# mrvollger/rustybam

Hardware: NVIDIA B200
Metric: lifted window-records/s (higher is better)
Workload: dtype u32/u64 (+f32 identities)

## Files before the change

### rustybam_b200/csrc/rb_kernels.cu

```cuda
#include <algorithm>
#include <cstdio>

#include "f32_fmt.cuh"
#include "lift_core.cuh"
#include "rb_kernels.cuh"
#include "rec_core.cuh"
#include "stream_core.cuh"

namespace rb {

__device__ __forceinline__ uint4 ld_nc_v4(const void* p) {
    uint4 r;
    asm volatile("ld.global.nc.L1::no_allocate.v4.u32 {%0,%1,%2,%3}, [%4];" : "=r"(r.x), "=r"(r.y), "=r"(r.z), "=r"(r.w) : "l"(p));
    return r;
}
__device__ __forceinline__ unsigned long long ld_volatile_u64(const unsigned long long* p) {
    unsigned long long v;
    asm volatile("ld.volatile.global.u64 %0, [%1];" : "=l"(v) : "l"(p));
    return v;
}
__device__ __forceinline__ uint32_t ld_volatile_u32(const uint32_t* p) {
    uint32_t v;
    asm volatile("ld.volatile.global.u32 %0, [%1];" : "=r"(v) : "l"(p));
    return v;
// ... 428 lines not shown
            __threadfence();
            x = payload_load(st == 2u ? &pre[idx] : &agg[idx]);
        }
        const unsigned stopm = __ballot_sync(0xffffffffu, st == 2u || x.flag);
        const int stop = stopm ? (__ffs(stopm) - 1) : 31;
        if (lane > stop) x = seg_identity();
#pragma unroll
        for (int d = 1; d < 32; d <<= 1) {
            const SegVal y = seg_shfl(x, (lane + d) & 31);
            if (lane + d < 32) x = seg_combine(y, x);
        }
        const SegVal tot = seg_shfl(x, 0);
        acc = seg_combine(tot, acc);
        if (stopm) break;
        look -= 32;
        if (look < 0) break;
    }
    if (lane == 0) {
        const SegVal incl = seg_combine(acc, mine);
        payload_store(&pre[b], incl);
        __threadfence();
        atomicExch(&state[b], 2u);
    }
    return acc;
}

__device__ __forceinline__ void st_b128(void* p, uint32_t a, uint32_t b, uint32_t c, uint32_t d) {
    const unsigned long long lo = ((unsigned long long)b << 32) | a, hi = ((unsigned long long)d << 32) | c;
    asm volatile("{\n .reg .b128 r;\n mov.b128 r, {%1, %2};\n st.relaxed.gpu.global.b128 [%0], r;\n}" ::"l"(p), "l"(lo), "l"(hi) : "memory");
}
__device__ __forceinline__ uint4 ld_b128(const void* p) {
    unsigned long long lo, hi;
    asm volatile("{\n .reg .b128 r;\n ld.relaxed.gpu.global.b128 r, [%2];\n mov.b128 {%0, %1}, r;\n}" : "=l"(lo), "=l"(hi) : "l"(p) : "memory");
    return make_uint4((uint32_t)lo, (uint32_t)(lo >> 32), (uint32_t)hi, (uint32_t)(hi >> 32));
}
__device__ __forceinline__ void slot_store(ScanPayload* slot, const SegVal& v, uint32_t tag) {
    const uint32_t* in = reinterpret_cast<const uint32_t*>(&v);
    const uint32_t aux = (in[11] & ~SUB_ABS) | (v.flag ? SUB_ABS : 0u);
    uint4* o = reinterpret_cast<uint4*>(slot);
    st_b128(o + 0, in[0], in[1], in[2], tag);
    st_b128(o + 1, in[3], in[4], in[5], tag);
    st_b128(o + 2, in[6], in[7], in[8], tag);
    st_b128(o + 3, in[9], in[10], aux, tag);
}
__device__ __forceinline__ uint32_t slot_load(const ScanPayload* slot, SegVal& v) {
    const uint4* p = reinterpret_cast<const uint4*>(slot);
    const uint4 a = ld_b128(p + 0), b = ld_b128(p + 1), c = ld_b128(p + 2), d = ld_b128(p + 3);
    if (a.w != b.w || b.w != c.w || c.w != d.w) return 0u;
    uint32_t* out = reinterpret_cast<uint32_t*>(&v);
    out[0] = a.x; out[1] = a.y; out[2] = a.z; out[3] = b.x; out[4] = b.y; out[5] = b.z;
    out[6] = c.x; out[7] = c.y; out[8] = c.z; out[9] = d.x; out[10] = d.y;
    out[11] = d.z & ~SUB_ABS;
    v.flag = (d.z & SUB_ABS) ? 1u : 0u;
    return a.w;
}
__device__ __forceinline__ SegVal lookback_seg2(ScanPayload* slots, uint64_t b, const SegVal& mine) {
    const int lane = threadIdx.x & 31;
    SegVal acc = seg_identity();
    if (b == 0) {
        if (lane == 0) slot_store(&slots[0], mine, 2u);
        return acc;
    }
    if (lane == 0) slot_store(&slots[b], mine, 1u);
    long long look = (long long)b - 1;
    for (;;) {
        const long long idx = look - lane;
        uint32_t st = 2u;
        SegVal x = seg_identity();
        if (idx >= 0) {
            do { st = slot_load(&slots[idx], x); } while (st == 0u);
        }
        const unsigned stopm = __ballot_sync(0xffffffffu, st == 2u || x.flag);
        const int stop = stopm ? (__ffs(stopm) - 1) : 31;
        if (lane > stop) x = seg_identity();
#pragma unroll
        for (int d = 1; d < 32; d <<= 1) {
            const SegVal y = seg_shfl(x, (lane + d) & 31);
            if (lane + d < 32) x = seg_combine(y, x);
        }
        const SegVal tot = seg_shfl(x, 0);
        acc = seg_combine(tot, acc);
        if (stopm) break;
        look -= 32;
        if (look < 0) break;
    }
    if (lane == 0) slot_store(&slots[b], seg_combine(acc, mine), 2u);
    return acc;
}

struct WinStaged {
    const uint32_t* s_ps;
    const uint32_t* s_pe;
    uint32_t js0, je0;
    __device__ __forceinline__ uint32_t ps(uint32_t j) const { return s_ps[j - js0]; }
    __device__ __forceinline__ uint32_t pe(uint32_t j) const { return s_pe[j - je0]; }
};
__device__ __forceinline__ void store_half(void* dst, const void* src) {
    const uint4* s4 = reinterpret_cast<const uint4*>(src);
    uint4* d4 = reinterpret_cast<uint4*>(dst);
#pragma unroll
    for (int k = 0; k < 4; k++) d4[k] = s4[k];
}

template <bool LIFT>
__global__ void __launch_bounds__(SMP_THREADS, LIFT ? 2 : RB_SMP_MINB)
k_scan_lift(const uint32_t* __restrict__ ops, const uint64_t* __restrict__ n_ops_dev, const uint32_t* __restrict__ heads,
            Ctr* __restrict__ samples, uint32_t* blk_state, ScanPayload* blk_agg, ScanPayload* blk_pre, unsigned int* ticket,
            LiftArgs la) {
    extern __shared__ __align__(16) uint32_t s_dyn[];
// ... 199 lines not shown
            SegRec sr;
            sr.eo0 = R.eo0; sr.eo1 = R.eo1; sr.wlo = R.wlo; sr.whi = R.whi;
            sr.s_lo = sr.e_lo = sr.wlo; sr.s_hi = sr.e_hi = sr.whi;
            if (sr.whi > sr.wlo) {
                sr.pair0 = la.pair_off[la.rec_rank[r]];
                const WinGlobal wg{la.w_st, la.w_en, R.t_st, R.t_en};
                uint32_t Tseg = 0;
                for (int j = jb; j < je; j++) {
                    const uint32_t w = my_ops[j];
                    if (is_ref(op_code(w))) Tseg += op_len(w);
                }
                stream_segment(v, sr, wg, k0, (uint32_t)(je - jb), [&](uint32_t j) { return my_ops[jb + (int)j]; }, base, Tseg, acc,
                               [&](uint64_t p, const HalfS& hh) { store_half(&la.hs[p], &hh); },
                               [&](uint64_t p, const HalfE& hh) { store_half(&la.he[p], &hh); });
            }
        }
        if (je >= nvalid) break;
        jb = je;
        r++;
        base = ctr_zero();
    }
}

#ifndef RB_SMP2_MINB
#define RB_SMP2_MINB 4
#endif
#ifndef RB_SMP2_MINB_NOSUBS
#define RB_SMP2_MINB_NOSUBS 5
#endif
template <bool LOCAL, bool NOSUBS = false>
__global__ void __launch_bounds__(SMP_THREADS, NOSUBS ? RB_SMP2_MINB_NOSUBS : RB_SMP2_MINB)
k_samples2(const uint32_t* __restrict__ ops, const uint64_t* __restrict__ n_ops_dev, const uint32_t* __restrict__ heads,
           Ctr* __restrict__ samples, uint32_t* blk_state, ScanPayload* blk_agg, ScanPayload* blk_pre, unsigned int* ticket,
           uint32_t no_subs_arg ) {
    const bool no_subs = NOSUBS || no_subs_arg != 0u;
    static_assert(SAMPLE == 32u, "k_samples2 walks 32-op chunks");
    extern __shared__ __align__(16) uint32_t s_dyn2[];
    uint4* s_ops4 = reinterpret_cast<uint4*>(s_dyn2);
    uint32_t* s_acc = s_dyn2 + SMP_THREADS * SAMPLE;
    __shared__ SegVal s_warp[SMP_THREADS / 32];
    __shared__ SegVal s_blk;
    __shared__ unsigned int s_b;
    const int tid = threadIdx.x, lane = tid & 31, warp = tid >> 5;
    const uint64_t n_ops = *n_ops_dev;
    if (!LOCAL) {
        if (tid == 0) s_b = atomicAdd(ticket, 1u);
        __syncthreads();
    }
    const uint64_t b = LOCAL ? (uint64_t)blockIdx.x : (uint64_t)s_b;
    const uint64_t op0 = b * (uint64_t)SMP_OPS;
    if (op0 >= n_ops && !(n_ops == 0 && b == 0)) {
        if (LOCAL && tid == 0) payload_store(&blk_agg[b], seg_identity());
        return;
    }

    {
        const uint4* src = reinterpret_cast<const uint4*>(ops + op0);
#pragma unroll
        for (int i = 0; i < (int)SAMPLE / 4; i++) {
            const uint32_t v4 = (uint32_t)i * SMP_THREADS + tid;
            uint4 x = make_uint4(0u, 0u, 0u, 0u);
            if (op0 + (uint64_t)v4 * 4u < n_ops) x = src[v4];
            const uint32_t row = v4 >> 3, u = v4 & 7u;
            s_ops4[row * 8u + (u ^ (row & 7u))] = x;
        }
    }
    __syncthreads();

    const uint64_t chunk = b * SMP_THREADS + tid;
    const uint64_t first = chunk << SAMPLE_LOG2;
    int nvalid = 0;
    if (first < n_ops) nvalid = (n_ops - first) < SAMPLE ? (int)(n_ops - first) : (int)SAMPLE;
    const uint32_t h = nvalid ? heads[first >> 5] : 0u;
    const uint32_t sw = (uint32_t)tid & 7u;
    const uint4* row = s_ops4 + (uint32_t)tid * 8u;
    auto op_at = [&](int j) { return reinterpret_cast<const uint32_t*>(&row[((uint32_t)j >> 2) ^ sw])[j & 3]; };
    uint32_t prev_code = 99u;
    if (nvalid) {
        if (tid > 0) prev_code = op_code(s_ops4[(uint32_t)(tid - 1) * 8u + (7u ^ ((uint32_t)(tid - 1) & 7u))].w);
        else if (first > 0) prev_code = op_code(ops[first - 1]);
    }
    SegVal mine = seg_identity();
    ClassAcc acc;
    acc.sum = s_acc + tid; acc.stride = SMP_THREADS;
    acc_reset(acc);
    uint32_t slowc = 0;
    auto store_sub = [&](const Ctr& sub, uint32_t k) {
        uint4* dst = reinterpret_cast<uint4*>(samples + chunk * SUBS + k);
        const uint32_t* w = reinterpret_cast<const uint32_t*>(&sub);
        dst[0] = make_uint4(w[0], w[1], w[2], w[3]);
        dst[1] = make_uint4(w[4], w[5], w[6], w[7]);
        dst[2] = make_uint4(w[8], w[9], w[10], w[11]);
    };
    if (nvalid == (int)SAMPLE && h == 0u) {
        uint32_t iev = 0, dev = 0, txt = 0, big = 0;
#pragma unroll
// ... 37 lines not shown
                    for (int t = j0; t < j; t++) ctr_add_op(sub, op_at(t));
                } else {
                    acc_flush(acc, sub);
                }
                sub.aux = (((h >> 1) & ((1u << j) - 1u)) != 0u) ? SUB_ABS : 0u;
                store_sub(sub, (uint32_t)(j >> SUB_LOG2));
            }
            const uint32_t code = op_code(w);
            slowc += (op_len(w) == 0u) | (op_len(w) >= ACC_BIG) | ((!head) & (code == prev_code));
            acc_add_op(acc, w);
            prev_code = code;
        }
        if (acc.big >= ACC_BIG) {
            int j0 = 0;
            for (int j = 0; j < nvalid; j++)
                if ((h >> j) & 1u) j0 = j;
            for (int j = j0; j < nvalid; j++) ctr_add_op(mine.c, op_at(j));
        } else {
            acc_flush(acc, mine.c);
        }
    }
    mine.c.aux = (mine.c.aux & AUX_OVF) | (slowc & AUX_CNT);
    mine.flag = (h != 0u);

    SegVal inc = mine;
#pragma unroll
    for (int d = 1; d < 32; d <<= 1) {
        const SegVal y = seg_shfl(inc, (lane - d) & 31);
        if (lane >= d) inc = seg_combine(y, inc);
    }
    if (lane == 31) s_warp[warp] = inc;
    SegVal exl = seg_shfl(inc, (lane - 1) & 31);
    if (lane == 0) exl = seg_identity();
    __syncthreads();
    SegVal wpre = seg_identity(), btot = seg_identity();
    if (LOCAL) {
        for (int k = 0; k < warp; k++) wpre = seg_combine(wpre, s_warp[k]);
        if (tid == SMP_THREADS - 1) payload_store(&blk_agg[b], seg_combine(wpre, inc));
        SegVal pre = seg_combine(wpre, exl);
        if (h & 1u) { pre.c = ctr_zero(); pre.flag = 1u; }
        if (nvalid) {
            pre.c.aux = (pre.c.aux & ~SUB_ABS) | (pre.flag ? SUB_ABS : 0u);
            samples[chunk * SUBS] = pre.c;
        }
        return;
    }
    if (warp == 0) {
#pragma unroll
        for (int k = 0; k < SMP_THREADS / 32; k++) btot = seg_combine(btot, s_warp[k]);
#if RB_SMP2_LB2
        const SegVal ex = lookback_seg2(blk_agg, b, btot);
#else
        const SegVal ex = lookback_seg(blk_state, blk_agg, blk_pre, b, btot);
#endif
        if (lane == 0) s_blk = ex;
    } else {
        for (int k = 0; k < warp; k++) wpre = seg_combine(wpre, s_warp[k]);
    }
    __syncthreads();
    SegVal pre = seg_combine(seg_combine(s_blk, wpre), exl);
    if (h & 1u) pre.c = ctr_zero();
    if (no_subs) pre.c.aux = (pre.c.aux & ~SUB_ABS) | SUB_ABS;
    if (nvalid) samples[chunk * SUBS] = pre.c;
}

constexpr uint32_t TS_NONE = 0xFFFFFFFFu;
__global__ void __launch_bounds__(256)
k_rec_heads(const uint8_t* __restrict__ text, const uint64_t* __restrict__ cigar_off, uint32_t n_rec, uint64_t* __restrict__ head_pos,
            uint32_t* tile_first) {
    const uint32_t r = blockIdx.x * blockDim.x + threadIdx.x;
    if (r >= n_rec) return;
    const uint64_t c = cigar_off[r], e = cigar_off[r + 1];
    uint64_t hp = ~0ull;
    const uint64_t lim = (e - c > 16u) ? c + 16u : e;
    for (uint64_t p = c; p < lim; p++)
        if (((uint32_t)text[p] - 48u) >= 10u) { hp = p; break; }
    head_pos[r] = hp;
    if (hp != ~0ull) atomicMin(&tile_first[hp / TOK_TILE], r);
}

#ifndef RB_TOKSCAN_MINB
#define RB_TOKSCAN_MINB 4
#endif
__global__ void __launch_bounds__(TOK_THREADS, RB_TOKSCAN_MINB)
k_tok_scan(const uint8_t* __restrict__ text, uint32_t* __restrict__ ops, unsigned long long* tile_state, unsigned int* ticket,
           ErrSlots err, uint32_t* misc_flags, const uint32_t* __restrict__ tile_first, const uint64_t* __restrict__ head_pos,
// ... 1883 lines not shown
        if (nb) put_op(&s_stage[warp][inc - nb], op_len(w), op_code(w));
        __syncwarp();
        uint8_t* dst = out_text + body_of(r0) + base;
        for (uint32_t i = lane; i < tot; i += 32) dst[i] = s_stage[warp][i];
        return;
    }
    if (k >= k1) return;
    const uint32_t r = rec_of(k);
    const uint64_t a = op_off[r];
    uint64_t j = a;
    uint32_t pos = 0;
    if (k0 > a) { j = k0; pos = samples[c * SUBS].TXT; }
    for (; j < k; j++) pos += ndigits32(op_len(ops[j])) + 1u;
    put_op(out_text + body_of(r) + pos, op_len(w), op_code(w));
}

static size_t samples2_smem() { return (size_t)(SMP_THREADS * SAMPLE + 9 * SMP_THREADS) * sizeof(uint32_t); }
static size_t scan_lift_smem(bool lift) {
    return (size_t)(SMP_THREADS * (SAMPLE + 1) + 9 * SMP_THREADS + (lift ? 2 * SL_WCAP : 0)) * sizeof(uint32_t);
}
int init_kernel_attrs() {
    cudaError_t e = cudaFuncSetAttribute(k_scan_lift<true>, cudaFuncAttributeMaxDynamicSharedMemorySize, (int)scan_lift_smem(true));
    if (e == cudaSuccess) e = cudaFuncSetAttribute(k_scan_lift<false>, cudaFuncAttributeMaxDynamicSharedMemorySize, (int)scan_lift_smem(false));
    if (e == cudaSuccess) e = cudaFuncSetAttribute(k_samples2<true>, cudaFuncAttributeMaxDynamicSharedMemorySize, (int)samples2_smem());
    if (e == cudaSuccess) e = cudaFuncSetAttribute(k_samples2<false>, cudaFuncAttributeMaxDynamicSharedMemorySize, (int)samples2_smem());
    if (e == cudaSuccess) e = cudaFuncSetAttribute(k_samples2<false, true>, cudaFuncAttributeMaxDynamicSharedMemorySize, (int)samples2_smem());
    if (e == cudaSuccess) e = cudaFuncSetAttribute(k_serialise, cudaFuncAttributeMaxDynamicSharedMemorySize, SER_CAP);
    if (e == cudaSuccess) e = cudaFuncSetAttribute(k_emit<false>, cudaFuncAttributeMaxDynamicSharedMemorySize, EMIT_DYN_BYTES);
    if (e == cudaSuccess) e = cudaFuncSetAttribute(k_emit<true>, cudaFuncAttributeMaxDynamicSharedMemorySize, EMIT_DYN_BYTES);
    return e == cudaSuccess ? 0 : -1;
}
__global__ void k_add_u64(unsigned long long* __restrict__ p, uint64_t n, unsigned long long delta) {
    const uint64_t i = (uint64_t)blockIdx.x * blockDim.x + threadIdx.x;
    if (i < n) p[i] += delta;
}
void launch_add_u64(uint64_t* p, uint64_t n, uint64_t delta, cudaStream_t s) {
    if (n == 0 || delta == 0) return;
    k_add_u64<<<(unsigned)((n + 255) / 256), 256, 0, s>>>(reinterpret_cast<unsigned long long*>(p), n, delta);
}
void launch_whole_text(const uint32_t* ops, const uint64_t* op_off, uint32_t n_rec, const RecInfo* recs, const Ctr* samples,
                       const uint64_t* line_off, uint8_t* out_text, uint64_t n_ops_bound, cudaStream_t s) {
    if (n_rec == 0 || n_ops_bound == 0 || out_text == nullptr) return;
    const uint64_t chunks = (n_ops_bound + SAMPLE - 1) / SAMPLE;
    k_whole_text<<<(unsigned)((chunks + WT_THREADS / 32 - 1) / (WT_THREADS / 32)), WT_THREADS, 0, s>>>(ops, op_off, n_rec, recs, samples,
                                                                                                    line_off, out_text);
}
void launch_tokenise(const uint8_t* text, uint64_t n_tiles, uint32_t* ops, unsigned long long* tile_state, unsigned int* ticket,
                     ErrSlots err, uint32_t* misc_flags, cudaStream_t s) {
    if (n_tiles == 0) return;
    k_tokenise<<<(unsigned)n_tiles, TOK_THREADS, 0, s>>>(text, ops, tile_state, ticket, err, misc_flags);
}
void launch_tok_scan(const uint8_t* text, uint64_t n_tiles, const uint64_t* cigar_off, uint32_t n_rec, uint32_t* ops,
                     unsigned long long* tile_state, unsigned int* ticket, ErrSlots err, uint32_t* misc_flags, uint32_t* tile_first,
                     uint64_t* head_pos, Ctr* samples, uint32_t* seg_state, ScanPayload* seg_agg, ScanPayload* seg_pre, cudaStream_t s) {
    if (n_tiles == 0) return;
    if (n_rec) k_rec_heads<<<(n_rec + 255) / 256, 256, 0, s>>>(text, cigar_off, n_rec, head_pos, tile_first);
    k_tok_scan<<<(unsigned)n_tiles, TOK_THREADS, 0, s>>>(text, ops, tile_state, ticket, err, misc_flags, tile_first, head_pos, n_rec,
                                                         samples, seg_state, seg_agg, seg_pre);
}
void launch_rec_ops(const uint8_t* text, const uint64_t* cigar_off, uint32_t n_rec, const unsigned long long* tile_state,
                    uint64_t* op_off, uint32_t* heads, ErrSlots err, cudaStream_t s) {
    const uint64_t warps = (uint64_t)n_rec + 1;
    k_rec_ops<<<(unsigned)((warps * 32 + 255) / 256), 256, 0, s>>>(text, cigar_off, n_rec, tile_state, op_off, heads, err);
}
void launch_scan_lift(bool lift, const uint32_t* ops, const uint64_t* n_ops_dev, uint64_t n_ops_bound, const uint32_t* heads,
                      Ctr* samples, uint32_t* blk_state, ScanPayload* blk_agg, ScanPayload* blk_pre, unsigned int* ticket,
                      LiftArgs la, cudaStream_t s, bool no_subs) {
    const uint64_t blocks = (n_ops_bound + SMP_OPS - 1) / SMP_OPS;
    if (blocks == 0) return;
    if (lift)
        k_scan_lift<true><<<(unsigned)blocks, SMP_THREADS, scan_lift_smem(true), s>>>(ops, n_ops_dev, heads, samples, blk_state, blk_agg,
                                                                                      blk_pre, ticket, la);
    else if (getenv("RB_OLD_SAMPLES"))
        k_scan_lift<false><<<(unsigned)blocks, SMP_THREADS, scan_lift_smem(false), s>>>(ops, n_ops_dev, heads, samples, blk_state,
                                                                                        blk_agg, blk_pre, ticket, la);
    else if (!getenv("RB_SAMPLES_LOCAL")) {
#if RB_SMP2_LB2
        cudaMemsetAsync(blk_agg, 0, blocks * sizeof(ScanPayload), s);
#endif
        if (no_subs)
            k_samples2<false, true><<<(unsigned)blocks, SMP_THREADS, samples2_smem(), s>>>(ops, n_ops_dev, heads, samples, blk_state, blk_agg, blk_pre,
                                                                                           ticket, 1u);
        else
            k_samples2<false><<<(unsigned)blocks, SMP_THREADS, samples2_smem(), s>>>(ops, n_ops_dev, heads, samples, blk_state, blk_agg, blk_pre, ticket,
                                                                                     0u);
    } else {
        k_samples2<true><<<(unsigned)blocks, SMP_THREADS, samples2_smem(), s>>>(ops, n_ops_dev, heads, samples, blk_state, blk_agg, blk_pre, ticket, 0u);
        k_blk_scan<<<1, 1024, 0, s>>>(n_ops_dev, blk_agg, blk_pre);
        const uint64_t chunks = (n_ops_bound + SAMPLE - 1) / SAMPLE;
        k_smp_fix<<<(unsigned)((chunks + 255) / 256), 256, 0, s>>>(n_ops_dev, blk_pre, samples);
    }
}
void launch_combine(uint64_t n_pairs, const uint64_t* pair_off, const uint32_t* rec_order, uint32_t n_rec, const RecInfo* recs,
                    const uint32_t* ops, WinView win, const uint64_t* names_off, const HalfS* hs, const HalfE* he, PairRes* res,
                    uint32_t* line_len, ErrSlots err, cudaStream_t s) {
    if (n_pairs == 0) return;
    k_combine<<<(unsigned)((n_pairs + 127) / 128), 128, 0, s>>>(n_pairs, pair_off, rec_order, n_rec, recs, ops, win, names_off, hs, he,
                                                                res, line_len, err);
}
void launch_check_clips(const uint32_t* ops, const uint64_t* op_off, uint32_t n_rec, ErrSlots err, cudaStream_t s) {
    if (n_rec == 0) return;
    k_check_clips<<<(n_rec + 127) / 128, 128, 0, s>>>(ops, op_off, n_rec, err);
}
void launch_rec_prep(int mode, RecInput in, const uint64_t* op_off, const uint32_t* ops, const Ctr* samples, WinView win,
                     RecInfo* recs, uint32_t* pair_cnt, StatsDev st, ErrSlots err, cudaStream_t s) {
    if (in.n_rec == 0) return;
    k_rec_prep<<<(in.n_rec + 127) / 128, 128, 0, s>>>(mode, in, op_off, ops, samples, win, recs, pair_cnt, st, err);
}
void launch_whole_rows(uint32_t n_rec, const RecInfo* recs, PairRes* res, uint32_t* line_len, uint64_t* pair_off, LiftPlan* plans,
                       cudaStream_t s) {
    k_whole_rows<<<n_rec / 128 + 1, 128, 0, s>>>(n_rec, recs, res, line_len, pair_off, plans);
}
void launch_pair_scan(const uint32_t* pair_cnt, const uint32_t* rec_order, uint32_t n_rec, uint64_t* pair_off, cudaStream_t s) {
    k_pair_scan<<<1, 1024, 0, s>>>(pair_cnt, rec_order, n_rec, pair_off);
// ... 189 lines not shown
```

### rustybam_b200/csrc/rb_kernels.cuh

```cuda
#pragma once
#include <cuda_runtime.h>

#include "lift_core.cuh"
#include "rb_common.cuh"
#include "trim_core.cuh"

namespace rb {

#ifndef RB_TOK_THREADS
#define RB_TOK_THREADS 256
#endif
constexpr int TOK_THREADS = RB_TOK_THREADS;
#ifndef RB_TOK_EARLY_PUBLISH
#define RB_TOK_EARLY_PUBLISH 1
#endif
constexpr int TOK_TILE = TOK_THREADS * 16;
constexpr int TEXT_FRONT_PAD = 16;
#ifndef RB_SMP_THREADS
#define RB_SMP_THREADS 256
#endif
constexpr int SMP_THREADS = RB_SMP_THREADS;
constexpr int SMP_OPS = SMP_THREADS * (int)SAMPLE;
constexpr int SL_WCAP = 2048;
#ifndef RB_LIFT_THREADS
#define RB_LIFT_THREADS 128
#endif
#ifndef RB_LIFT_CCAP
#define RB_LIFT_CCAP 96
#endif
#ifndef RB_LIFT_MINB
#define RB_LIFT_MINB 6
#endif
#ifndef RB_LIFT_STAGE_SMP
#define RB_LIFT_STAGE_SMP 1
#endif
#ifndef RB_LIFT_CHAIN
#define RB_LIFT_CHAIN 1
#endif
#ifndef RB_SMP2_LB2
#define RB_SMP2_LB2 0
#endif
#ifndef RB_SMP_MINB
#define RB_SMP_MINB 3
#endif
#ifndef RB_EMIT_MINB
#define RB_EMIT_MINB 6
#endif
#ifndef RB_EMIT_STAGE_TEXT
#define RB_EMIT_STAGE_TEXT 0
#endif
#ifndef RB_EMIT_DIRECT
#define RB_EMIT_DIRECT 1
#endif
#ifndef RB_EMIT_MID_TEXT
#define RB_EMIT_MID_TEXT 0
#endif
constexpr int LIFT_THREADS = RB_LIFT_THREADS;
constexpr int LIFT_CCAP = RB_LIFT_CCAP;
constexpr int LNS_THREADS = 256;
constexpr int SER_LINES = 128;
#ifndef RB_SER_CAP_KB
#define RB_SER_CAP_KB 26
#endif
// ... 44 lines not shown
    unsigned long long* rec;
};

int init_kernel_attrs();
void launch_add_u64(uint64_t* p, uint64_t n, uint64_t delta, cudaStream_t s);
void launch_tokenise(const uint8_t* text, uint64_t n_tiles, uint32_t* ops, unsigned long long* tile_state,
                     unsigned int* ticket, ErrSlots err, uint32_t* misc_flags, cudaStream_t s);
void launch_tok_scan(const uint8_t* text, uint64_t n_tiles, const uint64_t* cigar_off, uint32_t n_rec, uint32_t* ops,
                     unsigned long long* tile_state, unsigned int* ticket, ErrSlots err, uint32_t* misc_flags, uint32_t* tile_first,
                     uint64_t* head_pos, Ctr* samples, uint32_t* seg_state, ScanPayload* seg_agg, ScanPayload* seg_pre, cudaStream_t s);
void launch_rec_ops(const uint8_t* text, const uint64_t* cigar_off, uint32_t n_rec, const unsigned long long* tile_state,
                    uint64_t* op_off, uint32_t* heads, ErrSlots err, cudaStream_t s);
struct LiftArgs {
    const RecInfo* recs;
    const uint64_t* op_off;
    uint32_t n_rec;
    const uint32_t* rec_rank;
    const uint64_t* pair_off;
    const uint64_t* w_st;
    const uint64_t* w_en;
    HalfS* hs;
    HalfE* he;
};
void launch_scan_lift(bool lift, const uint32_t* ops, const uint64_t* n_ops_dev, uint64_t n_ops_bound, const uint32_t* heads,
                      Ctr* samples, uint32_t* blk_state, ScanPayload* blk_agg, ScanPayload* blk_pre, unsigned int* ticket,
                      LiftArgs la, cudaStream_t s, bool no_subs = false);
void launch_combine(uint64_t n_pairs, const uint64_t* pair_off, const uint32_t* rec_order, uint32_t n_rec, const RecInfo* recs,
                    const uint32_t* ops, WinView win, const uint64_t* names_off, const HalfS* hs, const HalfE* he, PairRes* res,
                    uint32_t* line_len, ErrSlots err, cudaStream_t s);
void launch_invert_ops(uint32_t* ops, const uint64_t* op_off, uint32_t n_rec, const uint8_t* strand, uint64_t n_ops_bound,
                       cudaStream_t s);
void launch_check_clips(const uint32_t* ops, const uint64_t* op_off, uint32_t n_rec, ErrSlots err, cudaStream_t s);
void launch_rec_prep(int mode, RecInput in, const uint64_t* op_off, const uint32_t* ops, const Ctr* samples, WinView win,
                     RecInfo* recs, uint32_t* pair_cnt, StatsDev st, ErrSlots err, cudaStream_t s);
void launch_pair_scan(const uint32_t* pair_cnt, const uint32_t* rec_order, uint32_t n_rec, uint64_t* pair_off, cudaStream_t s);
enum : uint32_t { PLAN_UNIFORM = 1u,
                  PLAN_FAST = 2u };
struct LiftPlan {
    uint32_t k0;
    uint32_t uniform;
    uint64_t c_lo, c_hi;
};
void launch_whole_text(const uint32_t* ops, const uint64_t* op_off, uint32_t n_rec, const RecInfo* recs, const Ctr* samples,
                       const uint64_t* line_off, uint8_t* out_text, uint64_t n_ops_bound, cudaStream_t s);
void launch_whole_rows(uint32_t n_rec, const RecInfo* recs, PairRes* res, uint32_t* line_len, uint64_t* pair_off, LiftPlan* plans,
                       cudaStream_t s);
void launch_lift_plan(uint64_t n_pairs, const uint64_t* pair_off, const uint32_t* rec_order, uint32_t n_rec, const RecInfo* recs,
                      const Ctr* samples, WinView win, LiftPlan* plans, cudaStream_t s, bool mark_fast = false);
void launch_lift(uint64_t n_pairs, const uint64_t* pair_off, const uint32_t* rec_order, uint32_t n_rec, const RecInfo* recs,
// ... 103 lines not shown
```

### rustybam_b200/csrc/rbcuda.cu

```cuda
#include <algorithm>
#include <chrono>
#include <condition_variable>
#include <cstdarg>
#include <cstdio>
#include <cstdlib>
#include <cstring>
#include <functional>
#include <mutex>
#include <string>
#include <thread>
#include <unordered_map>
#include <vector>

#include <sys/mman.h>

#include "../../include/rbcuda.h"
#include "name_intern.hpp"
#include "paf_parse_core.cuh"
#include "rb_kernels.cuh"
#include "rec_core.cuh"
#include "trim_rounds.hpp"

using namespace rb;

// ... 386 lines not shown
        KScope k(ctx, "k_tokenise");
        launch_tokenise(text, b->n_tiles, b->ops.as<uint32_t>(), b->tile_state.as<unsigned long long>(), sc + SC_TICKET_TOK, err,
                        sc + SC_MISC, s);
    }
    {
        KScope k(ctx, "k_rec_ops");
        launch_rec_ops(text, b->cigar_off.as<uint64_t>(), b->n_rec, b->tile_state.as<unsigned long long>(), b->op_off.as<uint64_t>(),
                       b->heads.as<uint32_t>(), err, s);
    }
    if (b->invert) {
        KScope k(ctx, "k_invert_ops");
        launch_invert_ops(b->ops.as<uint32_t>(), b->op_off.as<uint64_t>(), b->n_rec, b->strand.as<uint8_t>(), b->ops_bound, s);
    }
    CU(cudaGetLastError());
    return RB_OK;
}

int run_scan(rb_ctx* ctx, rb_batch* b, const LiftArgs* la, bool no_subs = false) {
    cudaStream_t s = ctx->stream;
    uint32_t* sc = ctx->scalars.as<uint32_t>();
    if (!la && b->have_samples) return RB_OK;
    {
        KScope k(ctx, la ? "k_scan_lift" : "k_samples");
        launch_scan_lift(la != nullptr, b->ops.as<uint32_t>(), b->op_off.as<uint64_t>() + b->n_rec, b->ops_bound, b->heads.as<uint32_t>(),
                         b->samples.as<Ctr>(), b->blk_state.as<uint32_t>(), b->blk_agg.as<ScanPayload>(), b->blk_pre.as<ScanPayload>(),
                         sc + SC_TICKET_SMP, la ? *la : LiftArgs{}, s, no_subs && !la);
    }
    CU(cudaGetLastError());
    return RB_OK;
}

}

extern "C" {

const char* rb_version(void) { return "rbcuda 0.1 (sm_100a)"; }

static constexpr uint64_t REG_PIECE = 1ull << 30;
static std::mutex g_reg_mu;
static std::vector<std::pair<void*, std::vector<void*>>> g_reg;

int rb_host_register(void* ptr, uint64_t nbytes) {
    if (!ptr || !nbytes) return RB_ERR_BAD_ARG;
    std::vector<void*> done;
    const uint64_t a0 = reinterpret_cast<uintptr_t>(ptr), a1 = a0 + nbytes;
    for (uint64_t a = a0; a < a1;) {
        uint64_t e = (a / REG_PIECE + 1) * REG_PIECE;
        if (e > a1) e = a1;
        if (cudaHostRegister(reinterpret_cast<void*>(a), e - a, cudaHostRegisterDefault) != cudaSuccess) {
// ... 330 lines not shown
        g.off.resize(nw + 1);
        g.off[0] = 0;
        for (uint32_t i = 0; i < nw; i++) g.off[i + 1] = g.off[i] + (W->ids_off[perm[i] + 1] - W->ids_off[perm[i]]);
        g.ids.resize(g.off[nw] + 1);
        for (uint32_t i = 0; i < nw; i++) {
            const uint32_t j = perm[i];
            memcpy(g.ids.data() + g.off[i], W->ids + W->ids_off[j], W->ids_off[j + 1] - W->ids_off[j]);
        }
        CU(cudaMemcpyAsync(b->w_ids_off.p, g.off.data(), (size_t)(nw + 1) * 8, cudaMemcpyHostToDevice, s));
        if (g.off[nw]) CU(cudaMemcpyAsync(b->w_ids.p, g.ids.data(), g.off[nw], cudaMemcpyHostToDevice, s));
    }
    b->busy = true;
    (void)R;
    return RB_OK;
}

static int ensure_rec_buffers(rb_ctx* ctx, rb_batch* b, uint32_t n) {
    CU(b->cigar_off.ensure((size_t)(n + 1) * 8));
    CU(b->cols64.ensure((size_t)n * 7 * 8 + 8));
    CU(b->strand.ensure(n + 8));
    CU(b->ids32.ensure((size_t)n * 2 * 4 + 8));
    CU(b->rec_order.ensure((size_t)n * 4 + 8));
    CU(b->rec_rank.ensure((size_t)n * 4 + 8));
    CU(b->ops.ensure(b->ops_bound * 4 + 64));
    CU(b->tile_state.ensure(b->n_tiles * 8));
    if (tok_scan_enabled()) {
        CU(b->tile_first.ensure(b->n_tiles * 4));
        CU(b->head_pos.ensure((size_t)(n + 1) * 8));
        CU(b->seg_state.ensure(b->n_tiles * 4));
        CU(b->seg_agg.ensure(b->n_tiles * sizeof(ScanPayload)));
        CU(b->seg_pre.ensure(b->n_tiles * sizeof(ScanPayload)));
    }
    CU(b->heads.ensure((b->ops_bound / SAMPLE + 2) * 4));
    CU(b->samples.ensure((b->ops_bound / SAMPLE + 2) * SUBS * sizeof(Ctr)));
    const size_t smp_blocks = b->ops_bound / SMP_OPS + 2;
    CU(b->blk_state.ensure(smp_blocks * 4));
    CU(b->blk_agg.ensure(smp_blocks * sizeof(ScanPayload)));
    CU(b->blk_pre.ensure(smp_blocks * sizeof(ScanPayload)));
    CU(b->op_off.ensure((size_t)(n + 1) * 8));
    CU(b->recs.ensure((size_t)n * sizeof(RecInfo) + 8));
    CU(b->pair_cnt.ensure((size_t)n * 4 + 8));
    CU(b->pair_off.ensure((size_t)(n + 1) * 8));
    return RB_OK;
}

static void emission_ranks(const uint32_t* tid, uint32_t n, uint32_t n_names, bool file_order, uint32_t* order, uint32_t* rank) {
    std::vector<int64_t> first(n_names, -1);
// ... 2212 lines not shown
```

Measured before the change: 447.4 million.

## Replace samples kernel with persistent TMA double-buffered warp-specialized pipeline

Replaces the one-block-per-tile k_samples2 scan with a persistent, occupancy-sized grid. Each block fetches tiles by ticket and loads them through 2D TMA bulk-tensor copies with 128B swizzle into double-buffered shared memory. A dedicated extra warp runs the decoupled lookback for tile i while the compute warps walk tile i+1, and the two sides hand off through named barriers and mbarriers. This hides load latency and lookback serialization, at the cost of more shared memory per block, extra barrier complexity, and host-side tensor-map encoding on every launch.

```diff
diff --git a/rustybam_b200/csrc/rb_kernels.cu b/rustybam_b200/csrc/rb_kernels.cu
--- a/rustybam_b200/csrc/rb_kernels.cu
+++ b/rustybam_b200/csrc/rb_kernels.cu
@@ -1,5 +1,7 @@
 #include <algorithm>
 #include <cstdio>
+#include <cuda.h>
+#include <cudaTypedefs.h>
 
 #include "f32_fmt.cuh"
 #include "lift_core.cuh"
@@ -474,69 +476,6 @@
         __threadfence();
         atomicExch(&state[b], 2u);
     }
-    return acc;
-}
-
-__device__ __forceinline__ void st_b128(void* p, uint32_t a, uint32_t b, uint32_t c, uint32_t d) {
-    const unsigned long long lo = ((unsigned long long)b << 32) | a, hi = ((unsigned long long)d << 32) | c;
-    asm volatile("{\n .reg .b128 r;\n mov.b128 r, {%1, %2};\n st.relaxed.gpu.global.b128 [%0], r;\n}" ::"l"(p), "l"(lo), "l"(hi) : "memory");
-}
-__device__ __forceinline__ uint4 ld_b128(const void* p) {
-    unsigned long long lo, hi;
-    asm volatile("{\n .reg .b128 r;\n ld.relaxed.gpu.global.b128 r, [%2];\n mov.b128 {%0, %1}, r;\n}" : "=l"(lo), "=l"(hi) : "l"(p) : "memory");
-    return make_uint4((uint32_t)lo, (uint32_t)(lo >> 32), (uint32_t)hi, (uint32_t)(hi >> 32));
-}
-__device__ __forceinline__ void slot_store(ScanPayload* slot, const SegVal& v, uint32_t tag) {
-    const uint32_t* in = reinterpret_cast<const uint32_t*>(&v);
-    const uint32_t aux = (in[11] & ~SUB_ABS) | (v.flag ? SUB_ABS : 0u);
-    uint4* o = reinterpret_cast<uint4*>(slot);
-    st_b128(o + 0, in[0], in[1], in[2], tag);
-    st_b128(o + 1, in[3], in[4], in[5], tag);
-    st_b128(o + 2, in[6], in[7], in[8], tag);
-    st_b128(o + 3, in[9], in[10], aux, tag);
-}
-__device__ __forceinline__ uint32_t slot_load(const ScanPayload* slot, SegVal& v) {
-    const uint4* p = reinterpret_cast<const uint4*>(slot);
-    const uint4 a = ld_b128(p + 0), b = ld_b128(p + 1), c = ld_b128(p + 2), d = ld_b128(p + 3);
-    if (a.w != b.w || b.w != c.w || c.w != d.w) return 0u;
-    uint32_t* out = reinterpret_cast<uint32_t*>(&v);
-    out[0] = a.x; out[1] = a.y; out[2] = a.z; out[3] = b.x; out[4] = b.y; out[5] = b.z;
-    out[6] = c.x; out[7] = c.y; out[8] = c.z; out[9] = d.x; out[10] = d.y;
-    out[11] = d.z & ~SUB_ABS;
-    v.flag = (d.z & SUB_ABS) ? 1u : 0u;
-    return a.w;
-}
-__device__ __forceinline__ SegVal lookback_seg2(ScanPayload* slots, uint64_t b, const SegVal& mine) {
-    const int lane = threadIdx.x & 31;
-    SegVal acc = seg_identity();
-    if (b == 0) {
-        if (lane == 0) slot_store(&slots[0], mine, 2u);
-        return acc;
-    }
-    if (lane == 0) slot_store(&slots[b], mine, 1u);
-    long long look = (long long)b - 1;
-    for (;;) {
-        const long long idx = look - lane;
-        uint32_t st = 2u;
-        SegVal x = seg_identity();
-        if (idx >= 0) {
-            do { st = slot_load(&slots[idx], x); } while (st == 0u);
-        }
-        const unsigned stopm = __ballot_sync(0xffffffffu, st == 2u || x.flag);
-        const int stop = stopm ? (__ffs(stopm) - 1) : 31;
-        if (lane > stop) x = seg_identity();
-#pragma unroll
-        for (int d = 1; d < 32; d <<= 1) {
-            const SegVal y = seg_shfl(x, (lane + d) & 31);
-            if (lane + d < 32) x = seg_combine(y, x);
-        }
-        const SegVal tot = seg_shfl(x, 0);
-        acc = seg_combine(tot, acc);
-        if (stopm) break;
-        look -= 32;
-        if (look < 0) break;
-    }
-    if (lane == 0) slot_store(&slots[b], seg_combine(acc, mine), 2u);
     return acc;
 }
 
@@ -782,56 +721,10 @@
     }
 }
 
-#ifndef RB_SMP2_MINB
-#define RB_SMP2_MINB 4
-#endif
-#ifndef RB_SMP2_MINB_NOSUBS
-#define RB_SMP2_MINB_NOSUBS 5
-#endif
-template <bool LOCAL, bool NOSUBS = false>
-__global__ void __launch_bounds__(SMP_THREADS, NOSUBS ? RB_SMP2_MINB_NOSUBS : RB_SMP2_MINB)
-k_samples2(const uint32_t* __restrict__ ops, const uint64_t* __restrict__ n_ops_dev, const uint32_t* __restrict__ heads,
-           Ctr* __restrict__ samples, uint32_t* blk_state, ScanPayload* blk_agg, ScanPayload* blk_pre, unsigned int* ticket,
-           uint32_t no_subs_arg ) {
-    const bool no_subs = NOSUBS || no_subs_arg != 0u;
-    static_assert(SAMPLE == 32u, "k_samples2 walks 32-op chunks");
-    extern __shared__ __align__(16) uint32_t s_dyn2[];
-    uint4* s_ops4 = reinterpret_cast<uint4*>(s_dyn2);
-    uint32_t* s_acc = s_dyn2 + SMP_THREADS * SAMPLE;
-    __shared__ SegVal s_warp[SMP_THREADS / 32];
-    __shared__ SegVal s_blk;
-    __shared__ unsigned int s_b;
-    const int tid = threadIdx.x, lane = tid & 31, warp = tid >> 5;
-    const uint64_t n_ops = *n_ops_dev;
-    if (!LOCAL) {
-        if (tid == 0) s_b = atomicAdd(ticket, 1u);
-        __syncthreads();
-    }
-    const uint64_t b = LOCAL ? (uint64_t)blockIdx.x : (uint64_t)s_b;
-    const uint64_t op0 = b * (uint64_t)SMP_OPS;
-    if (op0 >= n_ops && !(n_ops == 0 && b == 0)) {
-        if (LOCAL && tid == 0) payload_store(&blk_agg[b], seg_identity());
-        return;
-    }
-
-    {
-        const uint4* src = reinterpret_cast<const uint4*>(ops + op0);
-#pragma unroll
-        for (int i = 0; i < (int)SAMPLE / 4; i++) {
-            const uint32_t v4 = (uint32_t)i * SMP_THREADS + tid;
-            uint4 x = make_uint4(0u, 0u, 0u, 0u);
-            if (op0 + (uint64_t)v4 * 4u < n_ops) x = src[v4];
-            const uint32_t row = v4 >> 3, u = v4 & 7u;
-            s_ops4[row * 8u + (u ^ (row & 7u))] = x;
-        }
-    }
-    __syncthreads();
-
-    const uint64_t chunk = b * SMP_THREADS + tid;
+__device__ __forceinline__ SegVal smp_walk(const uint4* s_ops4, int tid, const uint32_t* __restrict__ ops, uint64_t chunk, int nvalid,
+                                           uint32_t h, bool no_subs, uint32_t* s_acc, Ctr* __restrict__ samples) {
+    static_assert(SAMPLE == 32u, "smp_walk walks 32-op chunks");
     const uint64_t first = chunk << SAMPLE_LOG2;
-    int nvalid = 0;
-    if (first < n_ops) nvalid = (n_ops - first) < SAMPLE ? (int)(n_ops - first) : (int)SAMPLE;
-    const uint32_t h = nvalid ? heads[first >> 5] : 0u;
     const uint32_t sw = (uint32_t)tid & 7u;
     const uint4* row = s_ops4 + (uint32_t)tid * 8u;
     auto op_at = [&](int j) { return reinterpret_cast<const uint32_t*>(&row[((uint32_t)j >> 2) ^ sw])[j & 3]; };
@@ -915,46 +808,186 @@
     }
     mine.c.aux = (mine.c.aux & AUX_OVF) | (slowc & AUX_CNT);
     mine.flag = (h != 0u);
-
+    return mine;
+}
+__device__ __forceinline__ SegVal smp_warp_scan(const SegVal& mine, SegVal& exl) {
+    const int lane = threadIdx.x & 31;
     SegVal inc = mine;
 #pragma unroll
     for (int d = 1; d < 32; d <<= 1) {
         const SegVal y = seg_shfl(inc, (lane - d) & 31);
         if (lane >= d) inc = seg_combine(y, inc);
     }
+    exl = seg_shfl(inc, (lane - 1) & 31);
+    if (lane == 0) exl = seg_identity();
+    return inc;
+}
+
+constexpr int SMP_PIPE_THREADS = SMP_THREADS + 32;
+constexpr uint32_t SMP_TILE_BYTES = SMP_OPS * 4u;
+struct SmpPipeSmem {
+    uint4 ops[2][SMP_THREADS * 8];
+    uint32_t acc[9 * SMP_THREADS];
+    SegVal warp[3][SMP_THREADS / 32];
+    SegVal blk[2];
+    unsigned long long bar[2];
+    uint32_t tick[2];
+};
+enum : int { NB_SCANNED = 1, NB_PREFIX = 3 };
+__device__ __forceinline__ void bar_arrive(int id, int n) { asm volatile("bar.arrive %0, %1;" ::"r"(id), "r"(n) : "memory"); }
+__device__ __forceinline__ void bar_sync(int id, int n) { asm volatile("bar.sync %0, %1;" ::"r"(id), "r"(n) : "memory"); }
+__device__ __forceinline__ void mbar_arrive(unsigned long long* bar) {
+    asm volatile("mbarrier.arrive.shared::cta.b64 _, [%0];" ::"r"(smem_u32(bar)) : "memory");
+}
+__device__ __forceinline__ void tma_load_2d(void* dst, const CUtensorMap* map, int c0, int c1, unsigned long long* bar) {
+    asm volatile("cp.async.bulk.tensor.2d.shared::cluster.global.tile.mbarrier::complete_tx::bytes [%0], [%1, {%2, %3}], [%4];"
+                 ::"r"(smem_u32(dst)), "l"(reinterpret_cast<uint64_t>(map)), "r"(c0), "r"(c1), "r"(smem_u32(bar))
+                 : "memory");
+}
+template <bool NOSUBS>
+__global__ void __launch_bounds__(SMP_PIPE_THREADS, 3)
+k_samples_pipe(const __grid_constant__ CUtensorMap ops_map, const uint32_t* __restrict__ ops, const uint64_t* __restrict__ n_ops_dev,
+               const uint32_t* __restrict__ heads, Ctr* __restrict__ samples, uint32_t* blk_state, ScanPayload* blk_agg,
+               ScanPayload* blk_pre, unsigned int* ticket) {
+    extern __shared__ __align__(1024) uint8_t s_pipe[];
+    SmpPipeSmem& S = *reinterpret_cast<SmpPipeSmem*>(s_pipe);
+    const int tid = threadIdx.x, lane = tid & 31, warp = tid >> 5;
+    const uint64_t n_ops = *n_ops_dev;
+    auto past_end = [&](uint64_t b) { return b != 0 && b * (uint64_t)SMP_OPS >= n_ops; };
+    auto fetch = [&](int st) {
+        const unsigned int b = atomicAdd(ticket, 1u);
+        S.tick[st] = b;
+        if (past_end(b)) {
+            mbar_arrive(&S.bar[st]);
+        } else {
+            mbar_expect_tx(&S.bar[st], SMP_TILE_BYTES);
+            tma_load_2d(&S.ops[st][0], &ops_map, 0, (int)(b * (unsigned)SMP_THREADS), &S.bar[st]);
+        }
+        return b;
+    };
+    if (tid == SMP_THREADS) {
+        mbar_init(&S.bar[0], 1);
+        mbar_init(&S.bar[1], 1);
+        fetch(0);
+        fetch(1);
+    }
+    __syncthreads();
+
+    if (warp < SMP_THREADS / 32) {
+        SegVal exl_p = seg_identity();
+        uint64_t chunk_p = 0;
+        bool valid_p = false, head_p = false;
+        auto store = [&](int j) {
+            SegVal wpre = seg_identity();
+            for (int k = 0; k < warp; k++) wpre = seg_combine(wpre, S.warp[j % 3][k]);
+            SegVal pre = seg_combine(seg_combine(S.blk[j & 1], wpre), exl_p);
+            if (head_p) pre.c = ctr_zero();
+            if (NOSUBS) pre.c.aux = (pre.c.aux & ~SUB_ABS) | SUB_ABS;
+            if (!valid_p) return;
+            if (NOSUBS) {
+                const uint32_t* w = reinterpret_cast<const uint32_t*>(&pre.c);
+                uint4* dst = reinterpret_cast<uint4*>(samples + chunk_p * SUBS);
+                dst[0] = make_uint4(w[0], w[1], w[2], w[3]);
+                dst[1] = make_uint4(w[4], w[5], w[6], w[7]);
+                dst[2] = make_uint4(w[8], w[9], w[10], w[11]);
+                dst[3] = make_uint4(0u, 0u, 0u, 0u);
+            } else {
+                samples[chunk_p * SUBS] = pre.c;
+            }
+        };
+        int i = 0;
+        for (;; i++) {
+            const int st = i & 1;
+            mbar_wait(&S.bar[st], (uint32_t)(i >> 1) & 1u);
+            const uint64_t b = S.tick[st];
+            if (past_end(b)) break;
+            const uint64_t chunk = b * SMP_THREADS + tid;
+            const uint64_t first = chunk << SAMPLE_LOG2;
+            int nvalid = 0;
+            if (first < n_ops) nvalid = (n_ops - first) < SAMPLE ? (int)(n_ops - first) : (int)SAMPLE;
+            const uint32_t h = nvalid ? heads[first >> 5] : 0u;
+            const SegVal mine = smp_walk(S.ops[st], tid, ops, chunk, nvalid, h, NOSUBS, S.acc, samples);
+            SegVal exl;
+            const SegVal inc = smp_warp_scan(mine, exl);
+            if (lane == 31) S.warp[i % 3][warp] = inc;
+            bar_arrive(NB_SCANNED + st, SMP_PIPE_THREADS);
+            if (i) {
+                bar_sync(NB_PREFIX + (st ^ 1), SMP_PIPE_THREADS);
+                store(i - 1);
+            }
+            exl_p = exl; chunk_p = chunk; valid_p = nvalid != 0; head_p = h & 1u;
+        }
+        if (i) {
+            bar_sync(NB_PREFIX + ((i - 1) & 1), SMP_PIPE_THREADS);
+            store(i - 1);
+        }
+    } else {
+        uint64_t b = S.tick[0], b_next = S.tick[1];
+        for (int i = 0; !past_end(b); i++) {
+            const int st = i & 1;
+            bar_sync(NB_SCANNED + st, SMP_PIPE_THREADS);
+            uint32_t b2 = (uint32_t)b_next;
+            if (lane == 0 && !past_end(b_next)) b2 = fetch(st);
+            b2 = __shfl_sync(0xffffffffu, b2, 0);
+            SegVal btot = seg_identity();
+#pragma unroll
+            for (int k = 0; k < SMP_THREADS / 32; k++) btot = seg_combine(btot, S.warp[i % 3][k]);
+            const SegVal ex = lookback_seg(blk_state, blk_agg, blk_pre, b, btot);
+            if (lane == 0) S.blk[st] = ex;
+            __syncwarp();
+            bar_arrive(NB_PREFIX + st, SMP_PIPE_THREADS);
+            b = b_next;
+            b_next = b2;
+        }
+    }
+}
+
+__global__ void __launch_bounds__(SMP_THREADS, 4)
+k_samples_local(const uint32_t* __restrict__ ops, const uint64_t* __restrict__ n_ops_dev, const uint32_t* __restrict__ heads,
+                Ctr* __restrict__ samples, ScanPayload* blk_agg) {
+    extern __shared__ __align__(16) uint32_t s_dyn2[];
+    uint4* s_ops4 = reinterpret_cast<uint4*>(s_dyn2);
+    uint32_t* s_acc = s_dyn2 + SMP_THREADS * SAMPLE;
+    __shared__ SegVal s_warp[SMP_THREADS / 32];
+    const int tid = threadIdx.x, lane = tid & 31, warp = tid >> 5;
+    const uint64_t n_ops = *n_ops_dev;
+    const uint64_t b = blockIdx.x;
+    const uint64_t op0 = b * (uint64_t)SMP_OPS;
+    if (op0 >= n_ops && !(n_ops == 0 && b == 0)) {
+        if (tid == 0) payload_store(&blk_agg[b], seg_identity());
+        return;
+    }
+    {
+        const uint4* src = reinterpret_cast<const uint4*>(ops + op0);
+#pragma unroll
+        for (int i = 0; i < (int)SAMPLE / 4; i++) {
+            const uint32_t v4 = (uint32_t)i * SMP_THREADS + tid;
+            uint4 x = make_uint4(0u, 0u, 0u, 0u);
+            if (op0 + (uint64_t)v4 * 4u < n_ops) x = src[v4];
+            const uint32_t row = v4 >> 3, u = v4 & 7u;
+            s_ops4[row * 8u + (u ^ (row & 7u))] = x;
+        }
+    }
+    __syncthreads();
+    const uint64_t chunk = b * SMP_THREADS + tid;
+    const uint64_t first = chunk << SAMPLE_LOG2;
+    int nvalid = 0;
+    if (first < n_ops) nvalid = (n_ops - first) < SAMPLE ? (int)(n_ops - first) : (int)SAMPLE;
+    const uint32_t h = nvalid ? heads[first >> 5] : 0u;
+    const SegVal mine = smp_walk(s_ops4, tid, ops, chunk, nvalid, h, false, s_acc, samples);
+    SegVal exl;
+    const SegVal inc = smp_warp_scan(mine, exl);
     if (lane == 31) s_warp[warp] = inc;
-    SegVal exl = seg_shfl(inc, (lane - 1) & 31);
-    if (lane == 0) exl = seg_identity();
     __syncthreads();
-    SegVal wpre = seg_identity(), btot = seg_identity();
-    if (LOCAL) {
-        for (int k = 0; k < warp; k++) wpre = seg_combine(wpre, s_warp[k]);
-        if (tid == SMP_THREADS - 1) payload_store(&blk_agg[b], seg_combine(wpre, inc));
-        SegVal pre = seg_combine(wpre, exl);
-        if (h & 1u) { pre.c = ctr_zero(); pre.flag = 1u; }
-        if (nvalid) {
-            pre.c.aux = (pre.c.aux & ~SUB_ABS) | (pre.flag ? SUB_ABS : 0u);
-            samples[chunk * SUBS] = pre.c;
-        }
-        return;
-    }
-    if (warp == 0) {
-#pragma unroll
-        for (int k = 0; k < SMP_THREADS / 32; k++) btot = seg_combine(btot, s_warp[k]);
-#if RB_SMP2_LB2
-        const SegVal ex = lookback_seg2(blk_agg, b, btot);
-#else
-        const SegVal ex = lookback_seg(blk_state, blk_agg, blk_pre, b, btot);
-#endif
-        if (lane == 0) s_blk = ex;
-    } else {
-        for (int k = 0; k < warp; k++) wpre = seg_combine(wpre, s_warp[k]);
-    }
-    __syncthreads();
-    SegVal pre = seg_combine(seg_combine(s_blk, wpre), exl);
-    if (h & 1u) pre.c = ctr_zero();
-    if (no_subs) pre.c.aux = (pre.c.aux & ~SUB_ABS) | SUB_ABS;
-    if (nvalid) samples[chunk * SUBS] = pre.c;
+    SegVal wpre = seg_identity();
+    for (int k = 0; k < warp; k++) wpre = seg_combine(wpre, s_warp[k]);
+    if (tid == SMP_THREADS - 1) payload_store(&blk_agg[b], seg_combine(wpre, inc));
+    SegVal pre = seg_combine(wpre, exl);
+    if (h & 1u) { pre.c = ctr_zero(); pre.flag = 1u; }
+    if (nvalid) {
+        pre.c.aux = (pre.c.aux & ~SUB_ABS) | (pre.flag ? SUB_ABS : 0u);
+        samples[chunk * SUBS] = pre.c;
+    }
 }
 
 constexpr uint32_t TS_NONE = 0xFFFFFFFFu;
@@ -2884,9 +2917,9 @@
 int init_kernel_attrs() {
     cudaError_t e = cudaFuncSetAttribute(k_scan_lift<true>, cudaFuncAttributeMaxDynamicSharedMemorySize, (int)scan_lift_smem(true));
     if (e == cudaSuccess) e = cudaFuncSetAttribute(k_scan_lift<false>, cudaFuncAttributeMaxDynamicSharedMemorySize, (int)scan_lift_smem(false));
-    if (e == cudaSuccess) e = cudaFuncSetAttribute(k_samples2<true>, cudaFuncAttributeMaxDynamicSharedMemorySize, (int)samples2_smem());
-    if (e == cudaSuccess) e = cudaFuncSetAttribute(k_samples2<false>, cudaFuncAttributeMaxDynamicSharedMemorySize, (int)samples2_smem());
-    if (e == cudaSuccess) e = cudaFuncSetAttribute(k_samples2<false, true>, cudaFuncAttributeMaxDynamicSharedMemorySize, (int)samples2_smem());
+    if (e == cudaSuccess) e = cudaFuncSetAttribute(k_samples_local, cudaFuncAttributeMaxDynamicSharedMemorySize, (int)samples2_smem());
+    if (e == cudaSuccess) e = cudaFuncSetAttribute(k_samples_pipe<false>, cudaFuncAttributeMaxDynamicSharedMemorySize, (int)sizeof(SmpPipeSmem));
+    if (e == cudaSuccess) e = cudaFuncSetAttribute(k_samples_pipe<true>, cudaFuncAttributeMaxDynamicSharedMemorySize, (int)sizeof(SmpPipeSmem));
     if (e == cudaSuccess) e = cudaFuncSetAttribute(k_serialise, cudaFuncAttributeMaxDynamicSharedMemorySize, SER_CAP);
     if (e == cudaSuccess) e = cudaFuncSetAttribute(k_emit<false>, cudaFuncAttributeMaxDynamicSharedMemorySize, EMIT_DYN_BYTES);
     if (e == cudaSuccess) e = cudaFuncSetAttribute(k_emit<true>, cudaFuncAttributeMaxDynamicSharedMemorySize, EMIT_DYN_BYTES);
@@ -2925,33 +2958,55 @@
     const uint64_t warps = (uint64_t)n_rec + 1;
     k_rec_ops<<<(unsigned)((warps * 32 + 255) / 256), 256, 0, s>>>(text, cigar_off, n_rec, tile_state, op_off, heads, err);
 }
-void launch_scan_lift(bool lift, const uint32_t* ops, const uint64_t* n_ops_dev, uint64_t n_ops_bound, const uint32_t* heads,
-                      Ctr* samples, uint32_t* blk_state, ScanPayload* blk_agg, ScanPayload* blk_pre, unsigned int* ticket,
-                      LiftArgs la, cudaStream_t s, bool no_subs) {
+static cudaError_t ops_tensor_map(CUtensorMap* map, const uint32_t* ops, uint64_t n_ops_bound) {
+    static PFN_cuTensorMapEncodeTiled_v12000 encode = [] {
+        void* fn = nullptr;
+        cudaDriverEntryPointQueryResult q;
+        if (cudaGetDriverEntryPointByVersion("cuTensorMapEncodeTiled", &fn, 12000, cudaEnableDefault, &q) != cudaSuccess ||
+            q != cudaDriverEntryPointSuccess)
+            fn = nullptr;
+        return reinterpret_cast<PFN_cuTensorMapEncodeTiled_v12000>(fn);
+    }();
+    if (!encode) return cudaErrorNotSupported;
+    const cuuint64_t dims[2] = {SAMPLE, (n_ops_bound + SAMPLE - 1) / SAMPLE}, strides[1] = {SAMPLE * 4u};
+    const cuuint32_t box[2] = {SAMPLE, (cuuint32_t)SMP_THREADS}, estr[2] = {1, 1};
+    const CUresult r = encode(map, CU_TENSOR_MAP_DATA_TYPE_UINT32, 2, const_cast<uint32_t*>(ops), dims, strides, box, estr,
+                              CU_TENSOR_MAP_INTERLEAVE_NONE, CU_TENSOR_MAP_SWIZZLE_128B, CU_TENSOR_MAP_L2_PROMOTION_L2_256B,
+                              CU_TENSOR_MAP_FLOAT_OOB_FILL_NONE);
+    return r == CUDA_SUCCESS ? cudaSuccess : cudaErrorInvalidValue;
+}
+cudaError_t launch_scan_lift(bool lift, const uint32_t* ops, const uint64_t* n_ops_dev, uint64_t n_ops_bound, const uint32_t* heads,
+                             Ctr* samples, uint32_t* blk_state, ScanPayload* blk_agg, ScanPayload* blk_pre, unsigned int* ticket,
+                             LiftArgs la, cudaStream_t s, bool no_subs) {
     const uint64_t blocks = (n_ops_bound + SMP_OPS - 1) / SMP_OPS;
-    if (blocks == 0) return;
-    if (lift)
+    if (blocks == 0) return cudaSuccess;
+    if (lift) {
         k_scan_lift<true><<<(unsigned)blocks, SMP_THREADS, scan_lift_smem(true), s>>>(ops, n_ops_dev, heads, samples, blk_state, blk_agg,
                                                                                       blk_pre, ticket, la);
-    else if (getenv("RB_OLD_SAMPLES"))
+    } else if (getenv("RB_OLD_SAMPLES")) {
         k_scan_lift<false><<<(unsigned)blocks, SMP_THREADS, scan_lift_smem(false), s>>>(ops, n_ops_dev, heads, samples, blk_state,
                                                                                         blk_agg, blk_pre, ticket, la);
-    else if (!getenv("RB_SAMPLES_LOCAL")) {
-#if RB_SMP2_LB2
-        cudaMemsetAsync(blk_agg, 0, blocks * sizeof(ScanPayload), s);
-#endif
-        if (no_subs)
-            k_samples2<false, true><<<(unsigned)blocks, SMP_THREADS, samples2_smem(), s>>>(ops, n_ops_dev, heads, samples, blk_state, blk_agg, blk_pre,
-                                                                                           ticket, 1u);
-        else
-            k_samples2<false><<<(unsigned)blocks, SMP_THREADS, samples2_smem(), s>>>(ops, n_ops_dev, heads, samples, blk_state, blk_agg, blk_pre, ticket,
-                                                                                     0u);
+    } else if (!getenv("RB_SAMPLES_LOCAL")) {
+        auto kern = no_subs ? k_samples_pipe<true> : k_samples_pipe<false>;
+        int dev = 0, sms = 0, per_sm = 0;
+        cudaError_t e = cudaGetDevice(&dev);
+        if (e == cudaSuccess) e = cudaDeviceGetAttribute(&sms, cudaDevAttrMultiProcessorCount, dev);
+        if (e == cudaSuccess) e = cudaOccupancyMaxActiveBlocksPerMultiprocessor(&per_sm, kern, SMP_PIPE_THREADS, sizeof(SmpPipeSmem));
+        if (e != cudaSuccess) return e;
+        uint64_t grid = (uint64_t)std::max(per_sm, 1) * (uint64_t)sms;
+        if (const char* cap = getenv("RB_SMP_GRID")) grid = std::min<uint64_t>(grid, (uint64_t)std::max(atoi(cap), 1));
+        grid = std::min(grid, blocks);
+        CUtensorMap map;
+        if ((e = ops_tensor_map(&map, ops, n_ops_bound)) != cudaSuccess) return e;
+        kern<<<(unsigned)grid, SMP_PIPE_THREADS, sizeof(SmpPipeSmem), s>>>(map, ops, n_ops_dev, heads, samples, blk_state, blk_agg,
+                                                                           blk_pre, ticket);
     } else {
-        k_samples2<true><<<(unsigned)blocks, SMP_THREADS, samples2_smem(), s>>>(ops, n_ops_dev, heads, samples, blk_state, blk_agg, blk_pre, ticket, 0u);
+        k_samples_local<<<(unsigned)blocks, SMP_THREADS, samples2_smem(), s>>>(ops, n_ops_dev, heads, samples, blk_agg);
         k_blk_scan<<<1, 1024, 0, s>>>(n_ops_dev, blk_agg, blk_pre);
         const uint64_t chunks = (n_ops_bound + SAMPLE - 1) / SAMPLE;
         k_smp_fix<<<(unsigned)((chunks + 255) / 256), 256, 0, s>>>(n_ops_dev, blk_pre, samples);
     }
+    return cudaGetLastError();
 }
 void launch_combine(uint64_t n_pairs, const uint64_t* pair_off, const uint32_t* rec_order, uint32_t n_rec, const RecInfo* recs,
                     const uint32_t* ops, WinView win, const uint64_t* names_off, const HalfS* hs, const HalfE* he, PairRes* res,
diff --git a/rustybam_b200/csrc/rb_kernels.cuh b/rustybam_b200/csrc/rb_kernels.cuh
--- a/rustybam_b200/csrc/rb_kernels.cuh
+++ b/rustybam_b200/csrc/rb_kernels.cuh
@@ -36,9 +36,6 @@
 #endif
 #ifndef RB_LIFT_CHAIN
 #define RB_LIFT_CHAIN 1
-#endif
-#ifndef RB_SMP2_LB2
-#define RB_SMP2_LB2 0
 #endif
 #ifndef RB_SMP_MINB
 #define RB_SMP_MINB 3
@@ -129,9 +126,9 @@
     HalfS* hs;
     HalfE* he;
 };
-void launch_scan_lift(bool lift, const uint32_t* ops, const uint64_t* n_ops_dev, uint64_t n_ops_bound, const uint32_t* heads,
-                      Ctr* samples, uint32_t* blk_state, ScanPayload* blk_agg, ScanPayload* blk_pre, unsigned int* ticket,
-                      LiftArgs la, cudaStream_t s, bool no_subs = false);
+cudaError_t launch_scan_lift(bool lift, const uint32_t* ops, const uint64_t* n_ops_dev, uint64_t n_ops_bound, const uint32_t* heads,
+                             Ctr* samples, uint32_t* blk_state, ScanPayload* blk_agg, ScanPayload* blk_pre, unsigned int* ticket,
+                             LiftArgs la, cudaStream_t s, bool no_subs = false);
 void launch_combine(uint64_t n_pairs, const uint64_t* pair_off, const uint32_t* rec_order, uint32_t n_rec, const RecInfo* recs,
                     const uint32_t* ops, WinView win, const uint64_t* names_off, const HalfS* hs, const HalfE* he, PairRes* res,
                     uint32_t* line_len, ErrSlots err, cudaStream_t s);
diff --git a/rustybam_b200/csrc/rbcuda.cu b/rustybam_b200/csrc/rbcuda.cu
--- a/rustybam_b200/csrc/rbcuda.cu
+++ b/rustybam_b200/csrc/rbcuda.cu
@@ -432,9 +432,9 @@
     if (!la && b->have_samples) return RB_OK;
     {
         KScope k(ctx, la ? "k_scan_lift" : "k_samples");
-        launch_scan_lift(la != nullptr, b->ops.as<uint32_t>(), b->op_off.as<uint64_t>() + b->n_rec, b->ops_bound, b->heads.as<uint32_t>(),
-                         b->samples.as<Ctr>(), b->blk_state.as<uint32_t>(), b->blk_agg.as<ScanPayload>(), b->blk_pre.as<ScanPayload>(),
-                         sc + SC_TICKET_SMP, la ? *la : LiftArgs{}, s, no_subs && !la);
+        CU(launch_scan_lift(la != nullptr, b->ops.as<uint32_t>(), b->op_off.as<uint64_t>() + b->n_rec, b->ops_bound, b->heads.as<uint32_t>(),
+                            b->samples.as<Ctr>(), b->blk_state.as<uint32_t>(), b->blk_agg.as<ScanPayload>(), b->blk_pre.as<ScanPayload>(),
+                            sc + SC_TICKET_SMP, la ? *la : LiftArgs{}, s, no_subs && !la));
     }
     CU(cudaGetLastError());
     return RB_OK;
@@ -811,7 +811,7 @@
     CU(b->ids32.ensure((size_t)n * 2 * 4 + 8));
     CU(b->rec_order.ensure((size_t)n * 4 + 8));
     CU(b->rec_rank.ensure((size_t)n * 4 + 8));
-    CU(b->ops.ensure(b->ops_bound * 4 + 64));
+    CU(b->ops.ensure((b->ops_bound + SAMPLE - 1) / SAMPLE * SAMPLE * 4 + 64));
     CU(b->tile_state.ensure(b->n_tiles * 8));
     if (tok_scan_enabled()) {
         CU(b->tile_first.ensure(b->n_tiles * 4));
```

Measured after the change: 456.6 million (median of 6 runs). 1.02x the previous value.
